# jramapuram/BYOL

Measured on NVIDIA H100. Metric: images/sec, higher is better.
Workload: dtype bf16

## Files before the change

byol_b200/csrc/capi.cu:

```cuda
#include <stdarg.h>
#include <stdio.h>

#include <atomic>
#include <map>
#include <mutex>
#include <utility>

#include "common.cuh"

namespace byol {

static thread_local char g_last_error[512] = "";

void set_last_error(const char* fmt, ...) {
  va_list ap;
  va_start(ap, fmt);
  vsnprintf(g_last_error, sizeof(g_last_error), fmt, ap);
  va_end(ap);
}

int check_launch(const char* what) {
  cudaError_t e = cudaGetLastError();
  if (e != cudaSuccess) {
    set_last_error("%s: launch failed: %s", what, cudaGetErrorString(e));
// ... 74 lines not shown
  const cuuint32_t elem_strides[5] = {1u, 1u, 1u, 1u, 1u};
  const CUresult r = encode(tm, CU_TENSOR_MAP_DATA_TYPE_BFLOAT16, (cuuint32_t)rank, const_cast<void*>(base), dims,
                            byte_strides, box, elem_strides, CU_TENSOR_MAP_INTERLEAVE_NONE, swizzle,
                            CU_TENSOR_MAP_L2_PROMOTION_L2_256B, CU_TENSOR_MAP_FLOAT_OOB_FILL_NONE);
  if (r != CUDA_SUCCESS) {
    char shape[384];
    int len = snprintf(shape, sizeof(shape), "%llu (box %u)", (unsigned long long)dims[0], box[0]);
    for (int i = 1; i < rank; ++i)
      len += snprintf(shape + len, sizeof(shape) - len, ", %llu (box %u, stride %llu B)", (unsigned long long)dims[i],
                      box[i], (unsigned long long)byte_strides[i - 1]);
    set_last_error("%s: cuTensorMapEncodeTiled failed (%d): dims %s, base %p", what, (int)r, shape, base);
    return -3;
  }
  return 0;
}

int tmap_2d(CUtensorMap* tm, const void* base, uint64_t rows, uint64_t cols, uint64_t ld, uint32_t box_rows,
            uint32_t box_cols, const char* what) {
  const uint64_t dims[2] = {cols, rows};
  const uint64_t strides[1] = {ld * sizeof(bf16)};
  const uint32_t box[2] = {box_cols, box_rows};
  return tmap_bf16(tm, base, 2, dims, strides, box,
                   box_cols == 64u ? CU_TENSOR_MAP_SWIZZLE_128B : CU_TENSOR_MAP_SWIZZLE_64B, what);
}

namespace {
struct FixScratch {
  int dev;
  cudaStream_t stream;
  Fix128* p;
  int64_t n;
  bool leased;
};
static FixScratch g_fix[256];
static int g_fix_count = 0;
}

Fix128* fix_scratch(cudaStream_t stream, int64_t n) {
  const int dev = device_slot();
  FixScratch* e = nullptr;
  for (int i = 0; i < g_fix_count; ++i)
    if (g_fix[i].dev == dev && g_fix[i].stream == stream) e = &g_fix[i];
  if (e == nullptr) {
    if (g_fix_count == 256) { set_last_error("fix_scratch: too many streams"); return nullptr; }
    e = &g_fix[g_fix_count++];
    e->dev = dev; e->stream = stream; e->p = nullptr; e->n = 0; e->leased = false;
// ... 139 lines not shown
```

byol_b200/csrc/common.cuh:

```cuda
#pragma once
#include <cuda.h>
#include <cuda_bf16.h>
#include <cuda_runtime.h>
#include <stdint.h>

namespace byol {

typedef __nv_bfloat16 bf16;

void set_last_error(const char* fmt, ...);
int check_launch(const char* what);

static constexpr int kMaxDevices = 64;
int device_slot();
int device_sm_count();

int smem_opt_in(const void* kernel, int bytes, const char* what);
int resident_blocks(const void* kernel, int threads, int smem_bytes, const char* what);

int tmap_bf16(CUtensorMap* tm, const void* base, int rank, const uint64_t* dims, const uint64_t* byte_strides,
              const uint32_t* box, CUtensorMapSwizzle swizzle, const char* what);
int tmap_2d(CUtensorMap* tm, const void* base, uint64_t rows, uint64_t cols, uint64_t ld, uint32_t box_rows,
            uint32_t box_cols, const char* what);

struct Fix128 {
  unsigned long long lo;
  long long hi;
  double spill;
};
static constexpr double kFixSplit = 1048576.0;
Fix128* fix_scratch(cudaStream_t stream, int64_t n);
int fix_done(cudaStream_t stream, int rc);
int fix_flush(Fix128* acc, float* dst, int64_t n, cudaStream_t stream);
int fix_flush_stats(Fix128* acc, float* col_sum, float* col_sqsum, int64_t n, cudaStream_t stream);

__device__ __forceinline__ void fix_add_words(Fix128* acc, unsigned long long lo, long long hi) {
  atomicAdd(&acc->lo, lo);
  atomicAdd(reinterpret_cast<unsigned long long*>(&acc->hi), (unsigned long long)hi);
}
template <class AddSpill>
__device__ __forceinline__ bool fix_split_spill(double& v, AddSpill add_spill) {
  if (!(fabs(v) < kFixSplit)) {
    const double big = isfinite(v) ? trunc(v * 0x1p-20) * 0x1p20 : v;
    add_spill(big);
    if (!isfinite(v)) return false;
    v -= big;
// ... 124 lines not shown
  asm volatile("fence.proxy.async.shared::cta;" ::: "memory");
}

__device__ __forceinline__ void cp_async16_zfill(uint32_t dst_smem, const void* src, bool valid) {
  uint32_t sz = valid ? 16u : 0u;
  asm volatile("cp.async.cg.shared.global [%0], [%1], 16, %2;" ::"r"(dst_smem), "l"(src), "r"(sz) : "memory");
}
__device__ __forceinline__ void cp_async_commit() { asm volatile("cp.async.commit_group;" ::: "memory"); }
template <int N>
__device__ __forceinline__ void cp_async_wait() {
  asm volatile("cp.async.wait_group %0;" ::"n"(N) : "memory");
}

__device__ __forceinline__ void tma_prefetch_desc(const CUtensorMap* tmap) {
  asm volatile("prefetch.tensormap [%0];" ::"l"(tmap) : "memory");
}
__device__ __forceinline__ void tma_load_2d(uint32_t dst_smem, const CUtensorMap* tmap, uint64_t* bar, int c0,
                                            int c1) {
  asm volatile(
      "cp.async.bulk.tensor.2d.shared::cluster.global.mbarrier::complete_tx::bytes [%0], [%1, {%3, %4}], [%2];"
      ::"r"(dst_smem), "l"(tmap), "r"(smem_u32(bar)), "r"(c0), "r"(c1)
      : "memory");
}

__device__ __forceinline__ void tma_store_2d(const CUtensorMap* tmap, uint32_t src_smem, int c0, int c1) {
  asm volatile("cp.async.bulk.tensor.2d.global.shared::cta.bulk_group [%0, {%2, %3}], [%1];" ::"l"(tmap),
               "r"(src_smem), "r"(c0), "r"(c1)
               : "memory");
}
__device__ __forceinline__ void tma_store_commit() { asm volatile("cp.async.bulk.commit_group;" ::: "memory"); }
__device__ __forceinline__ void tma_store_wait_read() {
  asm volatile("cp.async.bulk.wait_group.read 0;" ::: "memory");
}
__device__ __forceinline__ void tma_store_wait_read1() {
  asm volatile("cp.async.bulk.wait_group.read 1;" ::: "memory");
}
__device__ __forceinline__ void tma_store_wait_all() { asm volatile("cp.async.bulk.wait_group 0;" ::: "memory"); }

__device__ __forceinline__ void wg_fence() { asm volatile("wgmma.fence.sync.aligned;" ::: "memory"); }
__device__ __forceinline__ void wg_commit() { asm volatile("wgmma.commit_group.sync.aligned;" ::: "memory"); }
template <int N>
__device__ __forceinline__ void wg_wait() {
  asm volatile("wgmma.wait_group.sync.aligned %0;" ::"n"(N) : "memory");
}
template <int R>
__device__ __forceinline__ void wg_fence_acc(float (&d)[R]) {
// ... 179 lines not shown
```

byol_b200/csrc/conv_igemm.cu:

```cuda
#include <stdarg.h>
#include <stdio.h>
#include <stdlib.h>
#include <string.h>

#include "common.cuh"

namespace byol {

static constexpr int BM = 128;
static constexpr int BK = 64;
static constexpr int A_STAGE_BYTES = BM * 128;
static constexpr int GATHER_LAG = 2;

struct ConvGemmParams {
  const bf16* src;
  void* dst;
  const bf16* resid;
  const uint8_t* resid_mask;
  int resid_up;
  const float* resid_f32;
  const float* bias;
  float* col_sum;
  float* col_sqsum;
  Fix128* fx;
  int Nimg, Hs, Ws, C;
  int Ho, Wo;
  int KH, KW;
  int mul, base, dk, div;
  int M, Ndim, Kg;
  int ldc;
  int num_kb;
  int tiles_n;
  int out_fp32;
  int relu;
  int small_src;
  int local_stats;
  int fold;
  int parity;
  int Hh, Wh;
  int Mc;
  int ncls;
  int cls_list[4];
};

struct TileInfo {
  int m0, n0, nkb;
  int cls_idx, ph, pw, kh0, kw0, nkw;
};

template <bool GROUPED = false>
__device__ __forceinline__ TileInfo tile_info(const ConvGemmParams& p, int tile, int BN_) {
  TileInfo t;
  t.m0 = (tile / p.tiles_n) * BM;
  t.n0 = (tile % p.tiles_n) * BN_;
  t.nkb = p.num_kb;
  t.cls_idx = 0; t.ph = 0; t.pw = 0; t.kh0 = 0; t.kw0 = 0; t.nkw = p.KW;
  if (p.parity) {
    t.cls_idx = t.m0 / p.Mc;
    const int cls = p.cls_list[t.cls_idx];
    t.ph = cls >> 1;
    t.pw = cls & 1;
    t.kh0 = (t.ph + p.base) & 1;
    t.kw0 = (t.pw + p.base) & 1;
    const int nkh = (p.KH - t.kh0 + 1) >> 1;
    t.nkw = (p.KW - t.kw0 + 1) >> 1;
// ... 33 lines not shown
  static_assert(!H16 || A_TMA, "bf16 hand-off: plain GEMM only (no parity mode)");
  using L = SmemLayout<BN, STAGES, A_TMA, H16>;
  constexpr int EW = L::EW;
  constexpr int CPW = L::CPW;
  constexpr int MMA_WARP = 8;
  constexpr int TMA_WARP = MMA_WARP + 8;
  extern __shared__ __align__(1024) uint8_t smem_raw[];
  uint8_t* smem = (uint8_t*)(((uintptr_t)smem_raw + 1023) & ~(uintptr_t)1023);
  if (smem + L::NEEDED > smem_raw + L::TOTAL) __trap();
  uint8_t* smemA = smem + L::A_OFF;
  uint8_t* smemB = smem + L::B_OFF;
  uint64_t* full_bar = (uint64_t*)(smem + L::BAR_OFF);
  uint64_t* empty_bar = full_bar + STAGES;
  uint64_t* tfull_bar = empty_bar + STAGES;
  uint64_t* tempty_bar = tfull_bar + 1;
  uint64_t* ofull_bar = tempty_bar + 1;
  uint64_t* oempty_bar = ofull_bar + 2;
  uint8_t* stage_out = smem + L::STAGE_OUT_OFF;
  float* accbuf = reinterpret_cast<float*>(smem + L::ACC_OFF);

  const int warp = threadIdx.x >> 5;
  const int lane = threadIdx.x & 31;
  const int num_kb = p.num_kb;

  if (warp == TMA_WARP && lane == 0) {
    for (int s = 0; s < STAGES; ++s) {
      mbar_init(&full_bar[s], A_TMA ? 1u : 129u);
      mbar_init(&empty_bar[s], 2u);
    }
    mbar_init(tfull_bar, 256u);
    mbar_init(tempty_bar, (uint32_t)EW);
    for (int b = 0; b < 2; ++b) {
      mbar_init(&ofull_bar[b], 256u);
      mbar_init(&oempty_bar[b], (uint32_t)EW);
    }
    fence_mbar_init();
    tma_prefetch_desc(&tmapB);
    if (A_TMA) tma_prefetch_desc(&tmapA);
    if (!p.out_fp32) tma_prefetch_desc(&tmapC);
  }
  __syncthreads();

  if (warp < EW) {
    const bool do_stats = p.col_sum != nullptr;
    const int quarter = warp & 3;
    const int col_w0 = (warp >> 2) * (CPW * 32);
    const uint32_t stage_base0 = smem_u32(stage_out + warp * L::STAGE_PER_WARP);
    int sbuf = 0;
    constexpr int NACC = CPW;
    uint64_t cs1[NACC], cs2[NACC];
#pragma unroll
    for (int i = 0; i < NACC; ++i) { cs1[i] = 0ull; cs2[i] = 0ull; }
    int local = 0;
    int stat_n0 = -1;
    const bool local_stats = H16 && do_stats && p.local_stats;
    unsigned long long* lstats = reinterpret_cast<unsigned long long*>(smem + L::NEEDED);
    if (local_stats) {
      for (int i = threadIdx.x; i < 4 * p.Ndim; i += EW * 32) lstats[i] = 0ull;
      epilogue_bar_sync(EW * 32);
    }
    auto flush_stats = [&]() {
// ... 169 lines not shown
                         "r"(q.z), "r"(q.w)
                         : "memory");
          }
          fence_proxy_async_smem();
          __syncwarp();
          if (lane == 0) {
            tma_store_2d(&tmapC, stage_base, nbase, mrow0);
            tma_store_commit();
          }
          if (do_stats) stats_narrow(stage_base, lane, rows_valid, cs1[cl], cs2[cl]);
          if (L::NBUF == 2) sbuf ^= 1;
        }
      }
    }
    if (do_stats && stat_n0 >= 0) flush_stats();
    if (local_stats) {
      epilogue_bar_sync(EW * 32);
      for (int i = threadIdx.x; i < 2 * p.Ndim; i += EW * 32) {
        const unsigned long long lo = lstats[2 * i], hi = lstats[2 * i + 1];
        if ((lo | hi) != 0ull) fix_add_words(p.fx + i, lo, (long long)hi);
      }
    }
    if (lane == 0) tma_store_wait_all();
  } else if (!A_TMA && warp >= EW && warp < EW + 4) {
    const int tid = threadIdx.x - 128;
    const int chunk = tid & 7;
    const int row0 = tid >> 3;
    int it = 0;
    const bool fast = GROUPED || ((p.C % BK == 0) && (p.KH * p.KW <= 32) && p.small_src);
    for (int tile = blockIdx.x; tile < num_tiles; tile += gridDim.x) {
      const TileInfo ti = tile_info<GROUPED>(p, tile, BN);
      const int m0 = ti.m0;
      if (!GROUPED && p.fold) {
        uint32_t mask[8];
        int roff[8];
#pragma unroll
        for (int i = 0; i < 8; ++i) {
          const int m = m0 + row0 + 16 * i;
          mask[i] = 0u;
          roff[i] = 0;
          if (m < p.M) {
            const int ow = m % p.Wo;
            const int t = m / p.Wo;
            const int oh = t % p.Ho;
            const int n = t / p.Ho;
            const int bh = oh * p.mul + p.base, bw = ow * p.mul + p.base;
            const int sw = bw + chunk;
// ... 199 lines not shown
        }
        wg_commit();
        wg_wait<1>();
        if (leader && prev_s >= 0) mbar_arrive(&empty_bar[prev_s]);
        prev_s = s;
      }
      wg_wait<0>();
      wg_fence_acc(d);
      if (leader && prev_s >= 0) mbar_arrive(&empty_bar[prev_s]);
      if constexpr (H16) {
        const int buf = local & 1;
        mbar_wait(&oempty_bar[buf], (uint32_t)(((local >> 1) & 1) ^ 1));
        acc_store_bf16_sw64<BN>(smem_u32(stage_out + buf * L::OUT_TILE_BYTES) + (uint32_t)wg * 2 * (BN / 32) * 2048u, d);
        fence_proxy_async_smem();
        mbar_arrive(&ofull_bar[buf]);
      } else {
        mbar_wait(tempty_bar, (uint32_t)((local & 1) ^ 1));
        acc_store_smem<BN>(accbuf, L::ACC_LD, wg * 64, 0, d);
        mbar_arrive(tfull_bar);
      }
    }
  } else if (warp == TMA_WARP) {
    if (lane == 0) {
      constexpr uint32_t tx = (uint32_t)L::B_STAGE_BYTES + (A_TMA ? (uint32_t)A_STAGE_BYTES : 0u);
      int it = 0;
      for (int tile = blockIdx.x; tile < num_tiles; tile += gridDim.x) {
        const TileInfo ti = tile_info<GROUPED>(p, tile, BN);
        const int n0 = ti.n0;
        const int m0 = ti.m0;
        int kh = ti.kh0, kw = ti.kw0, cc = 0;
        for (int kb = 0; kb < ti.nkb; ++kb, ++it) {
          const int s = it % STAGES;
          const uint32_t ph = (it / STAGES) & 1;
          mbar_wait(&empty_bar[s], ph ^ 1);
          mbar_arrive_expect_tx(&full_bar[s], tx);
          int kcol = kb * BK;
          if (p.parity) {
            kcol = (kh * p.KW + kw) * (GROUPED ? BK : p.C) + cc;
            if (!GROUPED) cc += BK;
            if (GROUPED || cc >= p.C) { cc = 0; kw += 2; if (kw >= p.KW) { kw = ti.kw0; kh += 2; } }
          }
          tma_load_2d(smem_u32(smemB + s * L::B_STAGE_BYTES), &tmapB, &full_bar[s], kcol, n0);
          if (A_TMA) tma_load_2d(smem_u32(smemA + s * A_STAGE_BYTES), &tmapA, &full_bar[s], kb * BK, m0);
        }
      }
    }
    __syncwarp();
  }
}

struct WgradParams {
  const bf16* src;
  float* dw;
  int Nimg, Hs, Ws, C;
  int Ho, Wo;
  int KH, KW;
  int stride, pad;
  int M;
  int Cout, Cin_real;
  int tiles_co, tiles_n;
  int splits, kb_per_split, num_kb_total;
  int Cg;
  int groups;
  int fold_kw;
  int small_src;
  float* part;
  int64_t ndw;
  int terms, kb_per_term;
  int ldsrc;
  int dy_term;
  int src_term[6];
};

static constexpr int WG_KROWS = 64;
static constexpr int WG_A_STAGE = 2 * WG_KROWS * 128;

static constexpr int WG_THREADS = 13 * 32;

template <int BN, int STAGES, bool B_TMA, bool GROUPED = false>
__global__ void __launch_bounds__(WG_THREADS, 1)
conv_wgrad_kernel(const __grid_constant__ CUtensorMap tmapA, const __grid_constant__ CUtensorMap tmapB,
                  const WgradParams p) {
  static_assert(!GROUPED || (BN == 128 && !B_TMA), "grouped mode: two 64-channel chunks, gathered B operand");
  constexpr int NCH = BN / 64;
  constexpr int NMMA = GROUPED ? 64 : BN;
  constexpr int B_STAGE = NCH * WG_KROWS * 128;
  extern __shared__ uint8_t smem_raw[];
  uint8_t* smem = (uint8_t*)(((uintptr_t)smem_raw + 1023) & ~(uintptr_t)1023);
  uint8_t* smemA = smem;
  uint8_t* smemB = smem + STAGES * WG_A_STAGE;
  uint64_t* full_bar = (uint64_t*)(smemB + STAGES * B_STAGE);
  uint64_t* empty_bar = full_bar + STAGES;

  const int warp = __shfl_sync(0xffffffffu, (int)(threadIdx.x >> 5), 0);
  const int lane = threadIdx.x & 31;
  int bid = blockIdx.x;
  const int tile_n = bid % p.tiles_n;    bid /= p.tiles_n;
  const int tile_co = bid % p.tiles_co;  bid /= p.tiles_co;
  const int split = bid;
  const int co0 = tile_co * 128;
  const int n0 = tile_n * BN;
  const int kb_begin = split * p.kb_per_split;
  int kb_end = kb_begin + p.kb_per_split;
  if (kb_end > p.num_kb_total) kb_end = p.num_kb_total;
  const int nkb = kb_end - kb_begin;
  const int taps = p.KH * p.KW;

  if (warp == 12 && lane == 0) {
    for (int s = 0; s < STAGES; ++s) {
      mbar_init(&full_bar[s], B_TMA ? 1u : 129u);
      mbar_init(&empty_bar[s], 2u);
    }
    fence_mbar_init();
    tma_prefetch_desc(&tmapA);
    if (B_TMA) tma_prefetch_desc(&tmapB);
  }
  __syncthreads();

  if (warp < 4) {
    if (!B_TMA) {
      constexpr int CHUNKS = NCH * 8;
      constexpr int PER_THREAD = WG_KROWS * CHUNKS / 128;
      const int chunk = threadIdx.x % CHUNKS;
      const int rbase = (threadIdx.x / CHUNKS) * PER_THREAD;
      const int ch64 = chunk >> 3, c16 = chunk & 7;
      const int col = n0 + chunk * 8;
      const int group = col / p.Cg;
      const int cw = col - group * p.Cg;
      int kh, kw, ci;
      bool cvalid = group < p.groups;
      if (p.fold_kw) { kh = group; kw = cw >> 3; ci = 0; cvalid = cvalid && kw < p.KW; }
      else           { kh = group / p.KW; kw = group - kh * p.KW; ci = cw; }
      if (GROUPED) { ci += co0; cvalid = cvalid && ci < p.C; }
      const int dh = kh - p.pad, dw = kw - p.pad;
      const int64_t sC = (int64_t)p.stride * p.ldsrc;
      for (int it = 0; it < nkb; ++it) {
        const int kb = kb_begin + it;
        const int term = p.terms == 1 ? 0 : kb / p.kb_per_term;
        const int s = it % STAGES;
        const uint32_t ph = (it / STAGES) & 1;
        if (it >= GATHER_LAG) {
          cp_async_wait<GATHER_LAG - 1>();
          fence_proxy_async_smem();
// ... 89 lines not shown
      for (int h = 0; h < 2; ++h) {
        const int co = co0 + r0 + 8 * h;
        const int colb = n0 + 8 * j + 2 * (t & 3);
        const int group = colb / p.Cg;
        const int cw = colb - group * p.Cg;
        const float v0 = d[4 * j + 2 * h], v1 = d[4 * j + 2 * h + 1];
        if (co >= p.Cout || group >= p.groups) continue;
        if (p.fold_kw) {
          float* gp = p.dw + ((int64_t)co * p.Cin_real) * taps + group * p.KW;
#pragma unroll
          for (int e = 0; e < 2; ++e) {
            const int kwj = (cw + e) >> 3, cj = (cw + e) & 7;
            if (kwj < p.KW && cj < p.Cin_real) add(gp + (int64_t)cj * taps + kwj, e ? v1 : v0);
          }
        } else {
          float* gp = p.dw + ((int64_t)co * p.Cin_real) * taps + group;
          if (cw < p.Cin_real) add(gp + (int64_t)cw * taps, v0);
          if (cw + 1 < p.Cin_real) add(gp + (int64_t)(cw + 1) * taps, v1);
        }
      }
    }
  } else {
    if (lane == 0) {
      constexpr uint32_t tx = (uint32_t)WG_A_STAGE + (B_TMA ? (uint32_t)B_STAGE : 0u);
      for (int it = 0; it < nkb; ++it) {
        const int kb = kb_begin + it;
        const int term = p.terms == 1 ? 0 : kb / p.kb_per_term;
        const int row = (kb - term * p.kb_per_term) * WG_KROWS;
        const int col_a = co0 + term * p.dy_term;
        const int s = it % STAGES;
        const uint32_t ph = (it / STAGES) & 1;
        mbar_wait(&empty_bar[s], ph ^ 1);
        mbar_arrive_expect_tx(&full_bar[s], tx);
        const uint32_t a_base = smem_u32(smemA + s * WG_A_STAGE);
        tma_load_2d(a_base, &tmapA, &full_bar[s], col_a, row);
        tma_load_2d(a_base + WG_KROWS * 128, &tmapA, &full_bar[s], col_a + 64, row);
        if (B_TMA) {
          const uint32_t b_base = smem_u32(smemB + s * B_STAGE);
#pragma unroll
          for (int c = 0; c < NCH; ++c)
            tma_load_2d(b_base + c * (WG_KROWS * 128), &tmapB, &full_bar[s], n0 + 64 * c + p.src_term[term], row);
        }
      }
    }
    __syncwarp();
  }
}

bool gemm_fused_applicable(int M, int C, int Ndim, int ldw, int ldc);
int gemm_fused_launch(const void* src, const void* wt, void* dst, const void* resid, const void* resid_mask,
                      const float* bias, int M, int C, int Ndim, int ldw, int ldc, int relu, cudaStream_t stream);

bool patch_conv_applicable(int H, int W, int C, int Ndim, int KH, int KW, int stride, int pad, int out_fp32,
                           const float* bias, int64_t src_elems);
int patch_conv_launch(const void* src, const void* wt, void* dst, const void* resid, float* col_sum, float* col_sqsum,
                      int Nimg, int H, int W, int C, int Ndim, int ldw, int ldc, int flip, int relu, int sms,
                      cudaStream_t stream, int grouped = 0);

bool patch_wgrad_applicable(int H, int W, int C, int Cin_real, int Cout, int KH, int KW, int stride, int pad);
int patch_wgrad_launch(const void* x, const void* dy, float* dw, int Nimg, int H, int W, int C, int Cout, int sms,
                       cudaStream_t stream, int gs = 0);

template <int BN, int STAGES, bool A_TMA, bool GROUPED = false, bool H16 = false>
static int launch_igemm(const CUtensorMap& ta, const CUtensorMap& tb, const CUtensorMap& tc,
                        const ConvGemmParams& p, int tiles_m, cudaStream_t stream) {
  using L = SmemLayout<BN, STAGES, A_TMA, H16>;
  auto kern = conv_igemm_kernel<BN, STAGES, A_TMA, GROUPED, H16>;
  ConvGemmParams q = p;
  const int64_t local_bytes = 32 * (int64_t)p.Ndim;
  q.local_stats = (H16 && p.col_sum != nullptr && L::TOTAL + local_bytes <= 232448) ? 1 : 0;
  const int smem = L::TOTAL + (q.local_stats ? (int)local_bytes : 0);
  if (smem_opt_in((const void*)kern, smem, "conv_igemm_kernel") != 0) return -2;
  const int num_tiles = tiles_m * p.tiles_n;
  int grid = device_sm_count();
  if (grid > num_tiles) grid = num_tiles;
  kern<<<grid, IG_THREADS, smem, stream>>>(ta, tb, tc, q, num_tiles);
  return check_launch("conv_igemm_kernel");
}

}

using namespace byol;

static int conv_igemm_impl(const void* src, const void* wt, void* dst, const void* resid, const float* resid_f32,
                           const void* resid_mask, int resid_up, const float* bias, float* col_sum, float* col_sqsum,
                           int Nimg, int Hs, int Ws, int C, int Ho, int Wo, int Ndim, int KH, int KW, int stride,
                           int pad, int mode, int ldw, int ldc, int out_fp32, int relu, int force_gather,
                           cudaStream_t stream, int grouped = 0) {
  BYOL_CHECK_ARG(src && wt && dst, "byol_conv_igemm: null pointer");
  BYOL_CHECK_ARG(resid_f32 == nullptr || (out_fp32 && resid == nullptr && !resid_up),
                 "byol_conv_igemm: an fp32 residual needs an fp32 output and no other residual");
  BYOL_CHECK_ARG(C % 8 == 0 && C >= 8, "byol_conv_igemm: C=%d must be a multiple of 8", C);
  BYOL_CHECK_ARG(Ndim > 0 && (Ndim % 8 == 0 || (out_fp32 && resid == nullptr && col_sum == nullptr)),
                 "byol_conv_igemm: Ndim=%d must be a multiple of 8 (any width only for plain fp32 outputs)", Ndim);
  BYOL_CHECK_ARG(ldc >= Ndim && (ldc % 8 == 0 || out_fp32), "byol_conv_igemm: bad ldc=%d", ldc);
  BYOL_CHECK_ARG(!(out_fp32 && col_sum != nullptr), "byol_conv_igemm: fused statistics need a bf16 output");
  BYOL_CHECK_ARG((col_sum == nullptr) == (col_sqsum == nullptr), "byol_conv_igemm: need both statistics or none");
  BYOL_CHECK_ARG(stride == 1 || stride == 2, "byol_conv_igemm: stride %d unsupported", stride);
  BYOL_CHECK_ARG(mode == 0 || mode == 1, "byol_conv_igemm: bad mode %d", mode);
  const int64_t M64 = (int64_t)Nimg * Ho * Wo;
  BYOL_CHECK_ARG(M64 > 0 && M64 < (1ll << 31), "byol_conv_igemm: M out of range");
  BYOL_CHECK_ARG((int64_t)Nimg * Hs * Ws * C < (1ll << 40), "byol_conv_igemm: src too large");
  BYOL_CHECK_ARG(resid_mask == nullptr || (resid != nullptr && ldc % 8 == 0), "byol_conv_igemm: resid_mask without resid");
  BYOL_CHECK_ARG(!resid_up || (resid != nullptr && resid_mask == nullptr && Ho % 2 == 0 && Wo % 2 == 0 &&
                               !(mode == 1 && stride == 2)),
// ... 39 lines not shown
  int ncls = 0, cls_list[4];
  for (int cls = 0; cls < 4; ++cls) {
    const int ph = cls >> 1, pw = cls & 1;
    const int nkh = (KH - ((ph + pad) & 1) + 1) >> 1, nkw = (KW - ((pw + pad) & 1) + 1) >> 1;
    if (nkh > 0 && nkw > 0) cls_list[ncls++] = cls;
  }
  if (mode == 1 && stride == 2 && Ho % 2 == 0 && Wo % 2 == 0 && C % BK == 0 && p.small_src && KH <= 3 && KW <= 3 &&
      ((int64_t)Nimg * (Ho / 2) * (Wo / 2)) % BM == 0 && !out_fp32 && (resid == nullptr || ncls == 4)) {
    p.parity = 1;
    p.Hh = Ho / 2;
    p.Wh = Wo / 2;
    p.Mc = Nimg * p.Hh * p.Wh;
    p.ncls = ncls;
    for (int i = 0; i < ncls; ++i) p.cls_list[i] = cls_list[i];
    if (p.ncls < 4) {
      cudaError_t e = cudaMemsetAsync(dst, 0, (size_t)p.M * ldc * sizeof(bf16), stream);
      if (e != cudaSuccess) { set_last_error("byol_conv_igemm: memset failed: %s", cudaGetErrorString(e)); return -2; }
    }
    tiles_m = p.ncls * (p.Mc / BM);
  }
  const bool a_tma = !force_gather && KH == 1 && KW == 1 && stride == 1 && pad == 0;
  const bool h16 = a_tma && !out_fp32 && bias == nullptr && resid == nullptr && resid_mask == nullptr &&
                   resid_f32 == nullptr && !relu;

  CUtensorMap ta, tb, tc;
  memset(&ta, 0, sizeof(ta));
  if (tmap_2d(&tb, wt, (uint64_t)Ndim, (uint64_t)p.Kg, (uint64_t)ldw, (uint32_t)BN, 64u, "conv_igemm B") != 0) return -3;
  if (!out_fp32) {
    if (tmap_2d(&tc, dst, (uint64_t)p.M, (uint64_t)Ndim, (uint64_t)ldc, 32u, 32u, "conv_igemm C") != 0) return -3;
  } else {
    tc = tb;
  }
  if (a_tma) {
    if (tmap_2d(&ta, src, (uint64_t)p.M, (uint64_t)C, (uint64_t)C, (uint32_t)BM, 64u, "conv_igemm A") != 0) return -3;
  } else {
    ta = tb;
  }
  if (col_sum != nullptr) {
    p.fx = fix_scratch(stream, 2 * (int64_t)Ndim);
    if (p.fx == nullptr) return -2;
  }
  int rc;
  if (grouped) {
    rc = launch_igemm<64, 4, false, true>(ta, tb, tc, p, tiles_m, stream);
  } else if (BN == 128) {
    rc = h16     ? launch_igemm<128, 3, true, false, true>(ta, tb, tc, p, tiles_m, stream)
         : a_tma ? launch_igemm<128, 3, true>(ta, tb, tc, p, tiles_m, stream)
                 : launch_igemm<128, 3, false>(ta, tb, tc, p, tiles_m, stream);
  } else {
    rc = h16     ? launch_igemm<64, 3, true, false, true>(ta, tb, tc, p, tiles_m, stream)
         : a_tma ? launch_igemm<64, 3, true>(ta, tb, tc, p, tiles_m, stream)
                 : launch_igemm<64, 4, false>(ta, tb, tc, p, tiles_m, stream);
  }
  if (rc != 0 || col_sum == nullptr) return rc;
  return fix_flush_stats(p.fx, col_sum, col_sqsum, Ndim, stream);
}

extern "C" int byol_conv_igemm(const void* src, const void* wt, void* dst, const void* resid,
                               const void* resid_mask, int resid_up, const float* bias, float* col_sum, float* col_sqsum, int Nimg, int Hs, int Ws, int C, int Ho, int Wo,
                               int Ndim, int KH, int KW, int stride, int pad, int mode, int ldw, int ldc,
                               int out_fp32, int relu, int force_gather, cudaStream_t stream) {
  return conv_igemm_impl(src, wt, dst, resid, nullptr, resid_mask, resid_up, bias, col_sum, col_sqsum, Nimg, Hs, Ws, C,
                         Ho, Wo, Ndim, KH, KW, stride, pad, mode, ldw, ldc, out_fp32, relu, force_gather, stream);
}

static bool grouped_geometry_ok(const char* what, int Nimg, int H, int W, int C, int Ho, int Wo, int KH, int KW,
                                int stride, int pad) {
  if (Nimg <= 0 || H <= 0 || W <= 0 || C < 64 || C % 64 != 0 || KH != 3 || KW != 3 || pad != 1 ||
      (stride != 1 && stride != 2) || Ho != (H - 1) / stride + 1 || Wo != (W - 1) / stride + 1) {
    set_last_error("%s: unsupported geometry (N=%d H=%d W=%d C=%d Ho=%d Wo=%d KH=%d KW=%d stride=%d pad=%d): needs "
                   "C %% 64 == 0, 3x3, pad 1, stride 1 or 2", what, Nimg, H, W, C, Ho, Wo, KH, KW, stride, pad);
// ... 13 lines not shown
  BYOL_CHECK_ARG(x && wt && y, "byol_conv_fprop_grouped: null pointer");
  if (!grouped_geometry_ok("byol_conv_fprop_grouped", Nimg, H, W, C, Ho, Wo, KH, KW, stride, pad)) return -1;
  return conv_igemm_impl(x, wt, y, nullptr, nullptr, nullptr, 0, nullptr, col_sum, col_sqsum, Nimg, H, W, C, Ho, Wo,
                         C, KH, KW, stride, pad, 0, KH * KW * BK, C, 0, 0, 0, stream, 1);
}

extern "C" int byol_conv_dgrad_grouped(const void* dy, const void* wd, void* dx, int Nimg, int Ho, int Wo, int C,
                                       int H, int W, int KH, int KW, int stride, int pad, cudaStream_t stream) {
  BYOL_CHECK_ARG(dy && wd && dx, "byol_conv_dgrad_grouped: null pointer");
  if (!grouped_geometry_ok("byol_conv_dgrad_grouped", Nimg, H, W, C, Ho, Wo, KH, KW, stride, pad)) return -1;
  return conv_igemm_impl(dy, wd, dx, nullptr, nullptr, nullptr, 0, nullptr, nullptr, nullptr, Nimg, Ho, Wo, C, H, W,
                         C, KH, KW, stride, pad, 1, KH * KW * BK, C, 0, 0, 0, stream, 1);
}

extern "C" int byol_conv_dgrad_planes(const void* dy, const void* wd, float* dx, const float* resid_f32, int Nimg,
                                      int Hs, int Ws, int Cout, int H, int W, int Cin, int KH, int KW, int stride,
                                      int pad, int T, cudaStream_t stream) {
  BYOL_CHECK_ARG((T == 3 || T == 6) && Cout % 8 == 0 && Cin % 8 == 0, "byol_conv_dgrad_planes: bad args (T=%d Cout=%d Cin=%d)",
                 T, Cout, Cin);
  return conv_igemm_impl(dy, wd, dx, nullptr, resid_f32, nullptr, 0, nullptr, nullptr, nullptr, Nimg, Hs, Ws, T * Cout,
                         H, W, Cin, KH, KW, stride, pad, 1, KH * KW * T * Cout, Cin, 1, 0, 0, stream);
}

template <int BN, bool B_TMA, bool GROUPED = false>
static int launch_wgrad(const CUtensorMap& ta, const CUtensorMap& tb, const WgradParams& p, int grid,
                        cudaStream_t stream) {
  constexpr int STAGES = 4;
  constexpr int SMEM = STAGES * (WG_A_STAGE + (BN / 64) * WG_KROWS * 128) + 256 + 1024;
  auto kern = conv_wgrad_kernel<BN, STAGES, B_TMA, GROUPED>;
  if (smem_opt_in((const void*)kern, SMEM, "conv_wgrad_kernel") != 0) return -2;
  kern<<<grid, WG_THREADS, SMEM, stream>>>(ta, tb, p);
  return check_launch("conv_wgrad_kernel");
}

static int conv_wgrad_impl(const void* src, const void* dy, float* dw, int Nimg, int Hs, int Ws, int C, int Cin_real,
                           int Ho, int Wo, int Cout, int ldy, int KH, int KW, int stride, int pad, int force_gather,
                           int T, cudaStream_t stream, int gs = 0) {
  BYOL_CHECK_ARG(src && dy && dw, "byol_conv_wgrad: null pointer");
  if (ldy == 0) ldy = Cout;
  if (gs > 0) {
    if (!force_gather && Hs == Ho && Ws == Wo && patch_wgrad_applicable(Hs, Ws, C, C, Cout, KH, KW, stride, pad))
      return patch_wgrad_launch(src, dy, dw, Nimg, Hs, Ws, C, Cout, device_sm_count(), stream, gs);
  }
  BYOL_CHECK_ARG(C % 8 == 0 && ldy % 8 == 0 && ldy >= Cout && Cout > 0,
                 "byol_conv_wgrad: C=%d and the dy pitch %d must be multiples of 8 (Cout=%d)", C, ldy, Cout);
  BYOL_CHECK_ARG(Cin_real <= C, "byol_conv_wgrad: Cin_real > C");
  BYOL_CHECK_ARG(T == 0 || T == 3 || T == 6, "byol_conv_wgrad: bad T=%d", T);
  const int64_t M64 = (int64_t)Nimg * Ho * Wo;
  BYOL_CHECK_ARG(M64 > 0 && M64 < (1ll << 31), "byol_conv_wgrad: M out of range");
  if (T == 0 && !force_gather && ldy == Cout && Hs == Ho && Ws == Wo && patch_wgrad_applicable(Hs, Ws, C, Cin_real, Cout, KH, KW, stride, pad))
// ... 16 lines not shown
  p.fold_kw = (C == 8 && KW <= 8 && KW > 1) ? 1 : 0;
  BYOL_CHECK_ARG(p.fold_kw || C % 64 == 0 || KH * KW == 1, "byol_conv_wgrad: C=%d must be 8 (stem) or a multiple of 64", C);
  p.Cg = p.fold_kw ? 64 : gs > 0 ? 128 : C;
  p.groups = p.fold_kw ? KH : KH * KW;
  const int ncols = p.groups * p.Cg;
  const int BN = ncols > 64 ? 128 : 64;
  p.tiles_co = (Cout + 127) / 128;
  p.tiles_n = (ncols + BN - 1) / BN;
  p.kb_per_term = (p.M + WG_KROWS - 1) / WG_KROWS;
  p.num_kb_total = terms * p.kb_per_term;
  p.small_src = ((int64_t)Nimg * Hs * Ws * p.ldsrc < (1ll << 31) - (1ll << 24)) ? 1 : 0;
  const int taps = KH * KW;
  const int base_ctas = p.tiles_co * p.tiles_n;
  const int target_ctas = device_sm_count();
  int splits = target_ctas / base_ctas;
  int max_splits = (p.num_kb_total + 7) / 8;
  if (max_splits < 1) max_splits = 1;
  if (splits > max_splits) splits = max_splits;
  if (splits < 1) splits = 1;
  p.kb_per_split = (p.num_kb_total + splits - 1) / splits;
  p.splits = (p.num_kb_total + p.kb_per_split - 1) / p.kb_per_split;
  const int grid = base_ctas * p.splits;
  const bool b_tma = !force_gather && KH == 1 && KW == 1 && stride == 1 && pad == 0;

  BYOL_CHECK_ARG(!b_tma || C % 8 == 0, "byol_conv_wgrad: bad C");
  CUtensorMap ta, tb;
  const uint64_t dy_cols = T == 0 ? (uint64_t)Cout : (uint64_t)terms * ldy;
  if (tmap_2d(&ta, dy, (uint64_t)p.M, dy_cols, (uint64_t)terms * ldy, (uint32_t)WG_KROWS, 64u, "conv_wgrad dY") != 0)
    return -3;
  if (b_tma) {
    if (tmap_2d(&tb, src, (uint64_t)p.M, (uint64_t)p.ldsrc, (uint64_t)p.ldsrc, (uint32_t)WG_KROWS, 64u, "conv_wgrad X") != 0)
      return -3;
  } else {
    tb = ta;
  }
  p.ndw = (int64_t)Cout * Cin_real * taps;
  if (p.splits > 1) {
    p.part = part_scratch(stream, p.splits * p.ndw);
    if (p.part == nullptr) return -2;
  }
  const int rc = gs > 0 ? launch_wgrad<128, false, true>(ta, tb, p, grid, stream)
               : BN == 128 ? (b_tma ? launch_wgrad<128, true>(ta, tb, p, grid, stream) : launch_wgrad<128, false>(ta, tb, p, grid, stream))
                           : (b_tma ? launch_wgrad<64, true>(ta, tb, p, grid, stream) : launch_wgrad<64, false>(ta, tb, p, grid, stream));
  if (rc != 0 || p.splits == 1) return rc;
  return wgrad_reduce(p.part, p.splits, dw, p.ndw, stream);
}

extern "C" int byol_conv_wgrad_grouped(const void* x, const void* dy, float* dw, int Nimg, int H, int W, int C, int Cg,
                                       int Ho, int Wo, int KH, int KW, int stride, int pad, cudaStream_t stream) {
  BYOL_CHECK_ARG(x && dy && dw, "byol_conv_wgrad_grouped: null pointer");
  BYOL_CHECK_ARG(Cg >= 1 && Cg <= 64 && 64 % Cg == 0, "byol_conv_wgrad_grouped: Cg=%d must divide 64", Cg);
  if (!grouped_geometry_ok("byol_conv_wgrad_grouped", Nimg, H, W, C, Ho, Wo, KH, KW, stride, pad)) return -1;
  return conv_wgrad_impl(x, dy, dw, Nimg, H, W, C, Cg, Ho, Wo, C, C, KH, KW, stride, pad, 0, 0, stream, Cg);
}

extern "C" int byol_conv_wgrad(const void* src, const void* dy, float* dw, int Nimg, int Hs, int Ws, int C,
                               int Cin_real, int Ho, int Wo, int Cout, int ldy, int KH, int KW, int stride, int pad,
                               int force_gather, cudaStream_t stream) {
  return conv_wgrad_impl(src, dy, dw, Nimg, Hs, Ws, C, Cin_real, Ho, Wo, Cout, ldy, KH, KW, stride, pad, force_gather,
                         0, stream);
}

extern "C" int byol_conv_wgrad_planes(const void* src, const void* dy, float* dw, int Nimg, int Hs, int Ws, int C,
                                      int Cin_real, int Ho, int Wo, int Cout, int ldy, int KH, int KW, int stride,
                                      int pad, int T, cudaStream_t stream) {
  BYOL_CHECK_ARG(T == 3 || T == 6, "byol_conv_wgrad_planes: T=%d must be 3 or 6", T);
// ... 3 lines not shown
```

Measured before the change: 2664.

## Load conv activations via TMA im2col mode in forward and wgrad kernels

```diff
diff --git a/byol_b200/csrc/capi.cu b/byol_b200/csrc/capi.cu
--- a/byol_b200/csrc/capi.cu
+++ b/byol_b200/csrc/capi.cu
@@ -120,6 +120,46 @@
   const uint32_t box[2] = {box_cols, box_rows};
   return tmap_bf16(tm, base, 2, dims, strides, box,
                    box_cols == 64u ? CU_TENSOR_MAP_SWIZZLE_128B : CU_TENSOR_MAP_SWIZZLE_64B, what);
+}
+
+int tmap_im2col(CUtensorMap* tm, const void* base, int N, int H, int W, int C, int lo_h, int lo_w, int up_h, int up_w,
+                int stride, uint32_t pixels, const char* what) {
+  static const auto encode = []() -> decltype(&cuTensorMapEncodeIm2col) {
+    void* fn = nullptr;
+    cudaDriverEntryPointQueryResult q;
+    if (cudaGetDriverEntryPoint("cuTensorMapEncodeIm2col", &fn, cudaEnableDefault, &q) != cudaSuccess ||
+        q != cudaDriverEntryPointSuccess)
+      return nullptr;
+    return reinterpret_cast<decltype(&cuTensorMapEncodeIm2col)>(fn);
+  }();
+  if (encode == nullptr) {
+    set_last_error("%s: cuTensorMapEncodeIm2col entry point unavailable", what);
+    return -3;
+  }
+  auto corner_ok = [](int v) { return v >= -128 && v <= 127; };
+  if (((uintptr_t)base & 15u) != 0 || N <= 0 || H <= 0 || W <= 0 || C <= 0 || C % 64 != 0 || !corner_ok(lo_h) ||
+      !corner_ok(lo_w) || !corner_ok(up_h) || !corner_ok(up_w) || lo_h > H - 1 + up_h || lo_w > W - 1 + up_w ||
+      stride < 1 || stride > 8 || pixels == 0 || pixels > 1024) {
+    set_last_error("%s: no im2col map for base %p, [N=%d, H=%d, W=%d, C=%d], corners (%d, %d) / (%d, %d), stride %d, "
+                   "%u pixels: needs 16-byte alignment, C %% 64 == 0, corners in [-128, 127] around a non-empty box, "
+                   "stride 1..8 and 1..1024 pixels", what, base, N, H, W, C, lo_h, lo_w, up_h, up_w, stride, pixels);
+    return -3;
+  }
+  const cuuint64_t dims[4] = {(cuuint64_t)C, (cuuint64_t)W, (cuuint64_t)H, (cuuint64_t)N};
+  const cuuint64_t strides[3] = {(cuuint64_t)C * sizeof(bf16), (cuuint64_t)W * C * sizeof(bf16),
+                                 (cuuint64_t)H * W * C * sizeof(bf16)};
+  const int lower[2] = {lo_w, lo_h}, upper[2] = {up_w, up_h};
+  const cuuint32_t elem_strides[4] = {1u, (cuuint32_t)stride, (cuuint32_t)stride, 1u};
+  const CUresult r = encode(tm, CU_TENSOR_MAP_DATA_TYPE_BFLOAT16, 4u, const_cast<void*>(base), dims, strides, lower,
+                            upper, 64u, pixels, elem_strides, CU_TENSOR_MAP_INTERLEAVE_NONE, CU_TENSOR_MAP_SWIZZLE_128B,
+                            CU_TENSOR_MAP_L2_PROMOTION_L2_256B, CU_TENSOR_MAP_FLOAT_OOB_FILL_NONE);
+  if (r != CUDA_SUCCESS) {
+    set_last_error("%s: cuTensorMapEncodeIm2col failed (%d): [N=%d, H=%d, W=%d, C=%d], corners (%d, %d) / (%d, %d), "
+                   "stride %d, %u pixels, base %p", what, (int)r, N, H, W, C, lo_h, lo_w, up_h, up_w, stride, pixels,
+                   base);
+    return -3;
+  }
+  return 0;
 }
 
 namespace {
diff --git a/byol_b200/csrc/common.cuh b/byol_b200/csrc/common.cuh
--- a/byol_b200/csrc/common.cuh
+++ b/byol_b200/csrc/common.cuh
@@ -22,6 +22,8 @@
               const uint32_t* box, CUtensorMapSwizzle swizzle, const char* what);
 int tmap_2d(CUtensorMap* tm, const void* base, uint64_t rows, uint64_t cols, uint64_t ld, uint32_t box_rows,
             uint32_t box_cols, const char* what);
+int tmap_im2col(CUtensorMap* tm, const void* base, int N, int H, int W, int C, int lo_h, int lo_w, int up_h, int up_w,
+                int stride, uint32_t pixels, const char* what);
 
 struct Fix128 {
   unsigned long long lo;
@@ -192,6 +194,14 @@
       ::"r"(dst_smem), "l"(tmap), "r"(smem_u32(bar)), "r"(c0), "r"(c1)
       : "memory");
 }
+__device__ __forceinline__ void tma_load_im2col(uint32_t dst_smem, const CUtensorMap* tmap, uint64_t* bar, int c, int w,
+                                                int h, int n, uint16_t off_w, uint16_t off_h) {
+  asm volatile(
+      "cp.async.bulk.tensor.4d.shared::cluster.global.im2col.mbarrier::complete_tx::bytes"
+      " [%0], [%1, {%3, %4, %5, %6}], [%2], {%7, %8};"
+      ::"r"(dst_smem), "l"(tmap), "r"(smem_u32(bar)), "r"(c), "r"(w), "r"(h), "r"(n), "h"(off_w), "h"(off_h)
+      : "memory");
+}
 
 __device__ __forceinline__ void tma_store_2d(const CUtensorMap* tmap, uint32_t src_smem, int c0, int c1) {
   asm volatile("cp.async.bulk.tensor.2d.global.shared::cta.bulk_group [%0, {%2, %3}], [%1];" ::"l"(tmap),
diff --git a/byol_b200/csrc/conv_igemm.cu b/byol_b200/csrc/conv_igemm.cu
--- a/byol_b200/csrc/conv_igemm.cu
+++ b/byol_b200/csrc/conv_igemm.cu
@@ -2,6 +2,8 @@
 #include <stdio.h>
 #include <stdlib.h>
 #include <string.h>
+
+#include <algorithm>
 
 #include "common.cuh"
 
@@ -41,6 +43,8 @@
   int Mc;
   int ncls;
   int cls_list[4];
+  int a_im2col;
+  int im_lo_h, im_lo_w;
 };
 
 struct TileInfo {
@@ -120,10 +124,11 @@
   const int warp = threadIdx.x >> 5;
   const int lane = threadIdx.x & 31;
   const int num_kb = p.num_kb;
+  const bool a_im2col = !A_TMA && !GROUPED && p.a_im2col;
 
   if (warp == TMA_WARP && lane == 0) {
     for (int s = 0; s < STAGES; ++s) {
-      mbar_init(&full_bar[s], A_TMA ? 1u : 129u);
+      mbar_init(&full_bar[s], (A_TMA || a_im2col) ? 1u : 129u);
       mbar_init(&empty_bar[s], 2u);
     }
     mbar_init(tfull_bar, 256u);
@@ -134,7 +139,7 @@
     }
     fence_mbar_init();
     tma_prefetch_desc(&tmapB);
-    if (A_TMA) tma_prefetch_desc(&tmapA);
+    if (A_TMA || a_im2col) tma_prefetch_desc(&tmapA);
     if (!p.out_fp32) tma_prefetch_desc(&tmapC);
   }
   __syncthreads();
@@ -350,7 +355,7 @@
       }
     }
     if (lane == 0) tma_store_wait_all();
-  } else if (!A_TMA && warp >= EW && warp < EW + 4) {
+  } else if (!A_TMA && !a_im2col && warp >= EW && warp < EW + 4) {
     const int tid = threadIdx.x - 128;
     const int chunk = tid & 7;
     const int row0 = tid >> 3;
@@ -596,26 +601,45 @@
     }
   } else if (warp == TMA_WARP) {
     if (lane == 0) {
-      constexpr uint32_t tx = (uint32_t)L::B_STAGE_BYTES + (A_TMA ? (uint32_t)A_STAGE_BYTES : 0u);
+      const uint32_t tx = (uint32_t)L::B_STAGE_BYTES + ((A_TMA || a_im2col) ? (uint32_t)A_STAGE_BYTES : 0u);
       int it = 0;
       for (int tile = blockIdx.x; tile < num_tiles; tile += gridDim.x) {
         const TileInfo ti = tile_info<GROUPED>(p, tile, BN);
         const int n0 = ti.n0;
         const int m0 = ti.m0;
         int kh = ti.kh0, kw = ti.kw0, cc = 0;
+        const int kstep = p.parity ? 2 : 1;
+        int wn = 0, wh = 0, ww = 0;
+        if (a_im2col) {
+          if (p.parity) {
+            const int mc = m0 - ti.cls_idx * p.Mc;
+            const int t2 = mc / p.Wh;
+            ww = p.im_lo_w + mc % p.Wh;
+            wh = p.im_lo_h + t2 % p.Hh;
+            wn = t2 / p.Hh;
+          } else {
+            const int t2 = m0 / p.Wo;
+            ww = p.im_lo_w + (m0 % p.Wo) * p.mul;
+            wh = p.im_lo_h + (t2 % p.Ho) * p.mul;
+            wn = t2 / p.Ho;
+          }
+        }
         for (int kb = 0; kb < ti.nkb; ++kb, ++it) {
           const int s = it % STAGES;
           const uint32_t ph = (it / STAGES) & 1;
           mbar_wait(&empty_bar[s], ph ^ 1);
           mbar_arrive_expect_tx(&full_bar[s], tx);
-          int kcol = kb * BK;
-          if (p.parity) {
-            kcol = (kh * p.KW + kw) * (GROUPED ? BK : p.C) + cc;
-            if (!GROUPED) cc += BK;
-            if (GROUPED || cc >= p.C) { cc = 0; kw += 2; if (kw >= p.KW) { kw = ti.kw0; kh += 2; } }
-          }
+          const int kcol = p.parity ? (kh * p.KW + kw) * (GROUPED ? BK : p.C) + cc : kb * BK;
           tma_load_2d(smem_u32(smemB + s * L::B_STAGE_BYTES), &tmapB, &full_bar[s], kcol, n0);
           if (A_TMA) tma_load_2d(smem_u32(smemA + s * A_STAGE_BYTES), &tmapA, &full_bar[s], kb * BK, m0);
+          if (a_im2col) {
+            const int oh = p.parity ? ((ti.ph + p.base - kh) >> 1) : p.base + kh * p.dk;
+            const int ow = p.parity ? ((ti.pw + p.base - kw) >> 1) : p.base + kw * p.dk;
+            tma_load_im2col(smem_u32(smemA + s * A_STAGE_BYTES), &tmapA, &full_bar[s], cc, ww, wh, wn,
+                            (uint16_t)(ow - p.im_lo_w), (uint16_t)(oh - p.im_lo_h));
+          }
+          if (!GROUPED) cc += BK;
+          if (GROUPED || cc >= p.C) { cc = 0; kw += kstep; if (kw >= p.KW) { kw = ti.kw0; kh += kstep; } }
         }
       }
     }
@@ -644,6 +668,7 @@
   int ldsrc;
   int dy_term;
   int src_term[6];
+  int b_im2col;
 };
 
 static constexpr int WG_KROWS = 64;
@@ -679,20 +704,21 @@
   if (kb_end > p.num_kb_total) kb_end = p.num_kb_total;
   const int nkb = kb_end - kb_begin;
   const int taps = p.KH * p.KW;
+  const bool b_im2col = !B_TMA && !GROUPED && p.b_im2col;
 
   if (warp == 12 && lane == 0) {
     for (int s = 0; s < STAGES; ++s) {
-      mbar_init(&full_bar[s], B_TMA ? 1u : 129u);
+      mbar_init(&full_bar[s], (B_TMA || b_im2col) ? 1u : 129u);
       mbar_init(&empty_bar[s], 2u);
     }
     fence_mbar_init();
     tma_prefetch_desc(&tmapA);
-    if (B_TMA) tma_prefetch_desc(&tmapB);
+    if (B_TMA || b_im2col) tma_prefetch_desc(&tmapB);
   }
   __syncthreads();
 
   if (warp < 4) {
-    if (!B_TMA) {
+    if (!B_TMA && !b_im2col) {
       constexpr int CHUNKS = NCH * 8;
       constexpr int PER_THREAD = WG_KROWS * CHUNKS / 128;
       const int chunk = threadIdx.x % CHUNKS;
@@ -828,7 +854,7 @@
     }
   } else {
     if (lane == 0) {
-      constexpr uint32_t tx = (uint32_t)WG_A_STAGE + (B_TMA ? (uint32_t)B_STAGE : 0u);
+      const uint32_t tx = (uint32_t)WG_A_STAGE + ((B_TMA || b_im2col) ? (uint32_t)B_STAGE : 0u);
       for (int it = 0; it < nkb; ++it) {
         const int kb = kb_begin + it;
         const int term = p.terms == 1 ? 0 : kb / p.kb_per_term;
@@ -846,6 +872,20 @@
 #pragma unroll
           for (int c = 0; c < NCH; ++c)
             tma_load_2d(b_base + c * (WG_KROWS * 128), &tmapB, &full_bar[s], n0 + 64 * c + p.src_term[term], row);
+        }
+        if (b_im2col) {
+          const uint32_t b_base = smem_u32(smemB + s * B_STAGE);
+          const int t2 = row / p.Wo;
+          const int ww = (row % p.Wo) * p.stride - p.pad, wh = (t2 % p.Ho) * p.stride - p.pad, wn = t2 / p.Ho;
+#pragma unroll
+          for (int c = 0; c < NCH; ++c) {
+            const int col = n0 + 64 * c;
+            int group = col / p.Cg;
+            if (group >= p.groups) group = 0;
+            const int kh = group / p.KW, kw = group - kh * p.KW;
+            tma_load_im2col(b_base + c * (WG_KROWS * 128), &tmapB, &full_bar[s], col - (col / p.Cg) * p.Cg, ww, wh, wn,
+                            (uint16_t)kw, (uint16_t)kh);
+          }
         }
       }
     }
@@ -887,6 +927,9 @@
 }
 
 using namespace byol;
+
+static int im2col_upper(int lo, int n, int stride, int size) { return lo + (n - 1) * stride - (size - 1); }
+static bool im2col_corner_ok(int v) { return v >= -128 && v <= 127; }
 
 static int conv_igemm_impl(const void* src, const void* wt, void* dst, const void* resid, const float* resid_f32,
                            const void* resid_mask, int resid_up, const float* bias, float* col_sum, float* col_sqsum,
@@ -972,6 +1015,25 @@
   const bool a_tma = !force_gather && KH == 1 && KW == 1 && stride == 1 && pad == 0;
   const bool h16 = a_tma && !out_fp32 && bias == nullptr && resid == nullptr && resid_mask == nullptr &&
                    resid_f32 == nullptr && !relu;
+  int lo_h = p.base + (KH - 1) * (p.dk < 0 ? p.dk : 0), lo_w = p.base + (KW - 1) * (p.dk < 0 ? p.dk : 0);
+  int walk_h = Ho, walk_w = Wo, trav = p.mul;
+  if (p.parity) {
+    lo_h = lo_w = pad;
+    for (int i = 0; i < ncls; ++i) {
+      const int ph = cls_list[i] >> 1, pw = cls_list[i] & 1;
+      for (int kh = (ph + pad) & 1; kh < KH; kh += 2) lo_h = std::min(lo_h, (ph + pad - kh) >> 1);
+      for (int kw = (pw + pad) & 1; kw < KW; kw += 2) lo_w = std::min(lo_w, (pw + pad - kw) >> 1);
+    }
+    walk_h = p.Hh; walk_w = p.Wh; trav = 1;
+  }
+  const int up_h = im2col_upper(lo_h, walk_h, trav, Hs), up_w = im2col_upper(lo_w, walk_w, trav, Ws);
+  const bool a_im2col = !force_gather && !a_tma && !grouped && !p.fold && !out_fp32 && C % BK == 0 &&
+                        ((uintptr_t)src & 15u) == 0 && (mode == 0 || stride == 1 || p.parity) &&
+                        im2col_corner_ok(lo_h) && im2col_corner_ok(lo_w) && im2col_corner_ok(up_h) &&
+                        im2col_corner_ok(up_w);
+  p.a_im2col = a_im2col ? 1 : 0;
+  p.im_lo_h = lo_h;
+  p.im_lo_w = lo_w;
 
   CUtensorMap ta, tb, tc;
   memset(&ta, 0, sizeof(ta));
@@ -983,6 +1045,9 @@
   }
   if (a_tma) {
     if (tmap_2d(&ta, src, (uint64_t)p.M, (uint64_t)C, (uint64_t)C, (uint32_t)BM, 64u, "conv_igemm A") != 0) return -3;
+  } else if (a_im2col) {
+    if (tmap_im2col(&ta, src, Nimg, Hs, Ws, C, lo_h, lo_w, up_h, up_w, trav, (uint32_t)BM, "conv_igemm A im2col") != 0)
+      return -3;
   } else {
     ta = tb;
   }
@@ -994,9 +1059,10 @@
   if (grouped) {
     rc = launch_igemm<64, 4, false, true>(ta, tb, tc, p, tiles_m, stream);
   } else if (BN == 128) {
-    rc = h16     ? launch_igemm<128, 3, true, false, true>(ta, tb, tc, p, tiles_m, stream)
-         : a_tma ? launch_igemm<128, 3, true>(ta, tb, tc, p, tiles_m, stream)
-                 : launch_igemm<128, 3, false>(ta, tb, tc, p, tiles_m, stream);
+    rc = h16        ? launch_igemm<128, 3, true, false, true>(ta, tb, tc, p, tiles_m, stream)
+         : a_tma    ? launch_igemm<128, 3, true>(ta, tb, tc, p, tiles_m, stream)
+         : a_im2col ? launch_igemm<128, 4, false>(ta, tb, tc, p, tiles_m, stream)
+                    : launch_igemm<128, 3, false>(ta, tb, tc, p, tiles_m, stream);
   } else {
     rc = h16     ? launch_igemm<64, 3, true, false, true>(ta, tb, tc, p, tiles_m, stream)
          : a_tma ? launch_igemm<64, 3, true>(ta, tb, tc, p, tiles_m, stream)
@@ -1056,10 +1122,9 @@
                          H, W, Cin, KH, KW, stride, pad, 1, KH * KW * T * Cout, Cin, 1, 0, 0, stream);
 }
 
-template <int BN, bool B_TMA, bool GROUPED = false>
+template <int BN, bool B_TMA, bool GROUPED = false, int STAGES = 4>
 static int launch_wgrad(const CUtensorMap& ta, const CUtensorMap& tb, const WgradParams& p, int grid,
                         cudaStream_t stream) {
-  constexpr int STAGES = 4;
   constexpr int SMEM = STAGES * (WG_A_STAGE + (BN / 64) * WG_KROWS * 128) + 256 + 1024;
   auto kern = conv_wgrad_kernel<BN, STAGES, B_TMA, GROUPED>;
   if (smem_opt_in((const void*)kern, SMEM, "conv_wgrad_kernel") != 0) return -2;
@@ -1122,14 +1187,22 @@
   p.splits = (p.num_kb_total + p.kb_per_split - 1) / p.kb_per_split;
   const int grid = base_ctas * p.splits;
   const bool b_tma = !force_gather && KH == 1 && KW == 1 && stride == 1 && pad == 0;
+  const int up_h = im2col_upper(-pad, Ho, stride, Hs), up_w = im2col_upper(-pad, Wo, stride, Ws);
+  const bool b_im2col = !force_gather && !b_tma && T == 0 && gs == 0 && !p.fold_kw && C % 64 == 0 &&
+                        ((uintptr_t)src & 15u) == 0 && im2col_corner_ok(-pad) && im2col_corner_ok(up_h) &&
+                        im2col_corner_ok(up_w);
 
   BYOL_CHECK_ARG(!b_tma || C % 8 == 0, "byol_conv_wgrad: bad C");
   CUtensorMap ta, tb;
   const uint64_t dy_cols = T == 0 ? (uint64_t)Cout : (uint64_t)terms * ldy;
   if (tmap_2d(&ta, dy, (uint64_t)p.M, dy_cols, (uint64_t)terms * ldy, (uint32_t)WG_KROWS, 64u, "conv_wgrad dY") != 0)
     return -3;
+  p.b_im2col = b_im2col ? 1 : 0;
   if (b_tma) {
     if (tmap_2d(&tb, src, (uint64_t)p.M, (uint64_t)p.ldsrc, (uint64_t)p.ldsrc, (uint32_t)WG_KROWS, 64u, "conv_wgrad X") != 0)
+      return -3;
+  } else if (b_im2col) {
+    if (tmap_im2col(&tb, src, Nimg, Hs, Ws, C, -pad, -pad, up_h, up_w, stride, (uint32_t)WG_KROWS, "conv_wgrad X im2col") != 0)
       return -3;
   } else {
     tb = ta;
@@ -1139,9 +1212,14 @@
     p.part = part_scratch(stream, p.splits * p.ndw);
     if (p.part == nullptr) return -2;
   }
+  constexpr int IM2COL_STAGES = 6;
   const int rc = gs > 0 ? launch_wgrad<128, false, true>(ta, tb, p, grid, stream)
-               : BN == 128 ? (b_tma ? launch_wgrad<128, true>(ta, tb, p, grid, stream) : launch_wgrad<128, false>(ta, tb, p, grid, stream))
-                           : (b_tma ? launch_wgrad<64, true>(ta, tb, p, grid, stream) : launch_wgrad<64, false>(ta, tb, p, grid, stream));
+               : BN == 128 ? (b_tma      ? launch_wgrad<128, true>(ta, tb, p, grid, stream)
+                              : b_im2col ? launch_wgrad<128, false, false, IM2COL_STAGES>(ta, tb, p, grid, stream)
+                                         : launch_wgrad<128, false>(ta, tb, p, grid, stream))
+                           : (b_tma      ? launch_wgrad<64, true>(ta, tb, p, grid, stream)
+                              : b_im2col ? launch_wgrad<64, false, false, IM2COL_STAGES>(ta, tb, p, grid, stream)
+                                         : launch_wgrad<64, false>(ta, tb, p, grid, stream));
   if (rc != 0 || p.splits == 1) return rc;
   return wgrad_reduce(p.part, p.splits, dw, p.ndw, stream);
 }
```

New measurement: 2740, median of 6. 1.03x the previous value.
